# bplaum/gmerlin-avdecoder

Measured on AMD Instinct MI355X. Metric: RTjpeg 1080p decode frames/sec, higher is better.
Workload: dtype i32

## Files before the change

### gmerlin-avdecoder_amd/csrc/mi_rtjpeg.hip

```cpp
#include <hip/hip_runtime.h>
#include <stdarg.h>
#include <stdio.h>
#include <stdlib.h>
#include <string.h>

#include <algorithm>
#include <atomic>
#include <chrono>
#include <condition_variable>
#include <mutex>
#include <string>
#include <thread>
#include <vector>

#include "../../include/mi_rtjpeg.h"
#include "rtj_color_kernels.h"
#include "rtj_common.h"
#include "rtj_decode_chroma.h"
#include "rtj_decode_kernels.h"
#include "rtj_encode_kernels.h"
#include "rtj_format_kernels.h"
#include "rtj_index_kernels.h"
#include "rtj_runs_kernels.h"
#include "rtj_spec_kernels.h"
// ... 63 lines not shown
};

struct SpecIndex {
  bool on = false;
  uint64_t n = 0;
  std::vector<SpecChunkDev> h_chunks;
  std::vector<uint32_t> h_base;
  DevBuf<SpecChunkDev> chunks;
  DevBuf<uint32_t> rec;
  DevBuf<uint32_t> nrec;
  DevBuf<uint32_t> wstart;
  DevBuf<uint2> hand;
  DevBuf<uint2> fix;
  DevBuf<uint8_t> flag;
  DevBuf<uint32_t> nfix;
  DevBuf<uint32_t> base;
  DevBuf<uint32_t> ok;
  DevBuf<uint32_t> todo;
  DevBuf<uint32_t> state;
  uint64_t walkers_cap() const { return flag.cap; }
  uint64_t frames_cap() const { return todo.cap ? todo.cap - 2 : 0; }
};

struct SplitLists {
  DevBuf<uint2> list;
  DevBuf<uint32_t> cnt;
  PinnedBuf<uint32_t> h_mode_seen;
  uint32_t* d_mode_seen = nullptr;
  int flip = 0;
};
// ... 187 lines not shown
  auto spec_chunks_of = [](const FrameDev& f) -> uint32_t { return f.data_len / (uint32_t)kSpecChunk + 1u; };
  for (auto& f : p->h_frames) walkers += spec_chunks_of(f);
  sp.on = !p->sw.serial_index && !p->sw.emit_walk && (p->sw.spec_mode >= 1 || (p->sw.spec_mode != 0 && walkers >= kSpecMinWalkers));
  if (sp.on) {
    sp.h_chunks.clear();
    sp.h_base.assign(1, 0u);
    for (size_t i = 0; i < p->h_frames.size(); i++) {
      const uint32_t nsc = spec_chunks_of(p->h_frames[i]);
      for (uint32_t k = 0; k < nsc; k++) sp.h_chunks.push_back(SpecChunkDev{(uint32_t)i, k});
      sp.h_base.push_back((uint32_t)sp.h_chunks.size());
    }
    sp.n = sp.h_chunks.size();
    if (sp.n >= 0x7FFFFFFFull) sp.on = false;
  }
  if (!sp.on) return MI_RTJ_OK;
  const uint64_t frames = p->h_frames.size();
  if (sp.n > sp.walkers_cap() &&
      ((rc = dev_release(c, s, sp.chunks, sp.rec, sp.nrec, sp.wstart, sp.hand, sp.fix, sp.flag)) || (rc = sp.chunks.grow(c, sp.n, s)) ||
       (rc = sp.rec.grow(c, spec_bits_words(sp.n), s)) || (rc = sp.nrec.grow(c, sp.n, s)) || (rc = sp.wstart.grow(c, sp.n, s)) ||
       (rc = sp.hand.grow(c, sp.n, s)) || (rc = sp.fix.grow(c, sp.n, s)) || (rc = sp.flag.grow(c, sp.n, s, 64, true)) ||
       (rc = sp.nfix.grow(c, 1, s, 0, true))))
    return rc;
  if (frames > sp.frames_cap()) {
    if ((rc = dev_release(c, s, sp.base, sp.ok, sp.todo)) || (rc = sp.base.grow(c, frames + 1, s)) || (rc = sp.ok.grow(c, frames, s, 0, true)) ||
        (rc = sp.todo.grow(c, frames + 2, s)))
      return rc;
    HIPCHK(c, hipMemsetAsync(sp.todo + frames + 1, 0, sizeof(uint32_t), s));
    if ((rc = sp.state.grow(c, kSpecStWords, s, 0, true))) return rc;
  }
  HIPCHK(c, hipMemcpyAsync(sp.chunks, sp.h_chunks.data(), sizeof(SpecChunkDev) * sp.n, hipMemcpyHostToDevice, s));
  HIPCHK(c, hipMemcpyAsync(sp.base, sp.h_base.data(), sizeof(uint32_t) * sp.h_base.size(), hipMemcpyHostToDevice, s));
  HIPCHK(c, hipStreamSynchronize(s));
  return MI_RTJ_OK;
}

int plan_upload(mi_rtj_plan* p) {
  mi_rtj_ctx* c = p->ctx;
  HIPCHK(c, hipSetDevice(c->device));
  const int rc = p->own_frames.grow(c, (uint64_t)p->n, c->stream);
  if (rc != MI_RTJ_OK) return rc;
  p->d_frames = p->own_frames;
  HIPCHK(c, hipMemcpyAsync(p->own_frames, p->h_frames.data(), sizeof(FrameDev) * p->n, hipMemcpyHostToDevice, c->stream));
  return MI_RTJ_OK;
}
// ... 8 lines not shown

int plan_launch(mi_rtj_plan* p, const void* d_stream, void* d_out, int what = kLaunchAll, uint32_t dframe = 0,
                int dcount = -1) {
  mi_rtj_ctx* c = p->ctx;
  Launch L(p, (const uint8_t*)d_stream);
  if (p->fmt != MI_RTJ_FMT_YUV420)
    return launch_fmt(L, dim3(std::min<unsigned>((unsigned)p->n, 16384u)),
                      dim3(kFormats[p->fmt].parts * p->max_groups, (unsigned)p->n), (uint8_t*)d_out);
  int rc;
  if ((rc = launch_open(L, what)) != MI_RTJ_OK) return rc;
  if (what & kLaunchIndex) {
    unsigned rows = (unsigned)p->n;
    const bool spec = p->spec.on && !p->sw.serial_index;
    if (spec) {
      rows = std::min<unsigned>(rows, kSpecFallbackRows);
      const SpecGrids g{dim3((unsigned)((p->spec.n + 63) / 64)), dim3(p->n), dim3(kSpecRepairGrid)};
      if ((rc = stage_spec_index(L, g)) != MI_RTJ_OK) return rc;
    }
    ExactGrids g;
    g.walk = dim3(p->n);
    g.walk_todo = dim3(std::min<unsigned>((unsigned)p->n, 16384u));
    g.summarize = dim3(p->max_chunks, rows);
    g.resolve = dim3(spec ? std::min<unsigned>((unsigned)p->n, 1024u) : rows);
    g.emit = p->sw.emit_walk ? dim3(p->max_chunks, p->n) : dim3(p->max_chunks, rows);
    if ((rc = stage_exact_index(L, g)) != MI_RTJ_OK) return rc;
  }
  if ((rc = launch_hand_over(L, what)) != MI_RTJ_OK) return rc;
  if (!(what & kLaunchDecode)) {
    HIPCHK(c, hipGetLastError());
    return MI_RTJ_OK;
  }
// ... 591 lines not shown
```

### gmerlin-avdecoder_amd/csrc/rtj_host_stages.h

```cpp
#pragma once

namespace {

void drop_events(std::vector<Timed>& v) {
  for (auto& t : v) {
    if (t.a && t.owns_a) (void)hipEventDestroy(t.a);
    if (t.b) (void)hipEventDestroy(t.b);
  }
  v.clear();
}

struct KernelClock {
  mi_rtj_plan* p;
  hipStream_t cur;
  hipEvent_t prev = nullptr;
  Timed t;

  int begin() {
    if (!p->profile) return MI_RTJ_OK;
    t = Timed();
    if (prev) {
      t.a = prev;
      t.owns_a = false;
      return MI_RTJ_OK;
// ... 38 lines not shown
}
void launch_decode_fmt(int fmt, dim3 grid, hipStream_t s, const FrameDev* fr, const uint8_t* st, const QTab* lut, const uint32_t* blk, uint8_t* out) {
  if (fmt == MI_RTJ_FMT_YUV422) hipLaunchKernelGGL(k_decode_fmt<kFmtYUV422>, grid, dim3(kDecThreads), 0, s, fr, st, lut, blk, out);
  else hipLaunchKernelGGL(k_decode_fmt<kFmtGrey>, grid, dim3(kDecThreads), 0, s, fr, st, lut, blk, out);
}

struct WalkArgs {
  const FrameDev* frames;
  const SpecChunkDev* chunks;
  uint32_t total;
  const uint8_t* stream;
  const QTab* lut;
  uint32_t *recbits, *nrec, *wstart;
  uint2* hand;
  SpecReset rs;
};
#define WALK(kernel, ...) \
  hipLaunchKernelGGL(kernel, grid, dim3(64), 0, s, a.frames, a.chunks, a.total, a.stream, a.lut, a.recbits, a.nrec, a.wstart, a.hand, a.rs, ##__VA_ARGS__)
void launch_spec_walk(bool two_types, int spec_mode, uint32_t* state, dim3 grid, hipStream_t s, const WalkArgs& a) {
  if (state) {
    if (!two_types) WALK((k_spec_walk_any<false>), state);
    else WALK((k_spec_walk_any<true>), state);
  } else if (!two_types) {
    if (spec_mode == 1) WALK((k_spec_walk<false, kSpecLead>));
    if (spec_mode == 3) WALK((k_spec_walk<false, kSpecLeadLong>));
    if (spec_mode == 4) WALK((k_spec_walk<false, kSpecLeadVery>));
  } else {
    if (spec_mode == 1) WALK((k_spec_walk<true, kSpecLead>));
    if (spec_mode == 3) WALK((k_spec_walk<true, kSpecLeadLong>));
    if (spec_mode == 4) WALK((k_spec_walk<true, kSpecLeadVery>));
  }
}
#undef WALK

int launch_fmt(Launch& L, dim3 igrid, dim3 dgrid, uint8_t* out) {
  mi_rtj_plan* p = L.p;
  L.c->input_dirty = false;
// ... 33 lines not shown
  return MI_RTJ_OK;
}

struct SpecGrids {
  dim3 walk, verify, repair;
};
int stage_spec_index(Launch& L, const SpecGrids& g) {
  mi_rtj_plan* p = L.p;
  SpecIndex& s = p->spec;
  const QTab* lut = L.c->d_lut;
  const int mode = p->sw.spec_mode;
  const bool no_policy = mode == 1 || mode == 3 || mode == 4;
  L.state = no_policy ? nullptr : s.state.p;
  L.ntodo = s.todo;
  L.todo = s.todo + 1;
  STAGE_CHK(L.clk.begin());
  launch_spec_walk(!p->one_block_type, mode, L.state, g.walk, L.is,
                   WalkArgs{p->d_frames, s.chunks, (uint32_t)s.n, L.st, lut, s.rec, s.nrec, s.wstart, s.hand, SpecReset{s.nfix, s.todo, s.flag}});
  STAGE_CHK(L.clk.end(MI_RTJ_K_SPEC_WALK));
  STAGE_CHK(L.clk.begin());
  for (int pass = 1; pass <= 2; pass++) {
    hipLaunchKernelGGL(k_spec_verify, g.verify, dim3(kSpecVerThreads), 0, L.is, p->d_frames, s.base, lut, s.rec, s.nrec, L.blk,
                       s.ok, s.todo + 1, s.todo, L.state, s.wstart, s.hand, s.fix, s.nfix, s.flag, pass);
    if (pass == 1)
      hipLaunchKernelGGL(k_spec_repair, g.repair, dim3(64), 0, L.is, p->d_frames, s.chunks, L.st, lut, s.rec, s.nrec, s.wstart,
                         s.hand, s.fix, s.nfix, s.flag, (uint32_t)s.n, L.state);
  }
  STAGE_CHK(L.clk.end(MI_RTJ_K_SPEC_VERIFY));
  if (L.state)
    hipLaunchKernelGGL(k_spec_policy, dim3(1), dim3(256), 0, L.is, (uint32_t)p->n, (uint32_t)s.n, s.todo, s.nfix, L.state, p->sw.serial_min);
  return MI_RTJ_OK;
}

struct ExactGrids {
  dim3 walk, walk_todo, summarize, resolve, emit;
};
int stage_exact_index(Launch& L, const ExactGrids& g) {
  mi_rtj_plan* p = L.p;
  const QTab* lut = L.c->d_lut;
  const ChunkIndex& ch = p->chunk;
  if (p->sw.serial_index) {
// ... 151 lines not shown
```

### gmerlin-avdecoder_amd/csrc/rtj_host_switches.h

```cpp
#pragma once
#include <stdint.h>
#include <stdlib.h>
#include <string.h>

namespace mirtj {

static inline const char* exp_env(const char* name) {
#ifdef MIRTJ_EXPERIMENTS
  return getenv(name);
#else
  (void)name;
  return nullptr;
#endif
}

enum PlanKind { kPlanBatch = 0, kPlanOnePacket, kPlanSessionSlot, kPlanSessionGroup };

struct PlanSwitches {
  bool serial_index = false;
  bool emit_walk = false;
  int spec_mode = -1;
  uint32_t dec_slots = 0;
  int rotate = -1;
  uint32_t serial_min = 4096;
  int split = -1;
  bool overlap_set = false;
  int overlap = 0;
};

static inline PlanSwitches plan_switches_from_env(PlanKind kind) {
  PlanSwitches s;
  const char* v = getenv("MI_RTJ_INDEX");
  s.serial_index = v && strcmp(v, "serial") == 0;
  v = getenv("MI_RTJ_EMIT");
  s.emit_walk = v && strcmp(v, "walk") == 0;
  if (kind == kPlanSessionSlot || kind == kPlanSessionGroup) {
    s.spec_mode = 0;
    return s;
  }
  if ((v = getenv("MI_RTJ_SPEC"))) s.spec_mode = atoi(v);
  if (kind != kPlanBatch) return s;
  if ((v = getenv("MI_RTJ_DEC_SLOTS"))) s.dec_slots = (uint32_t)atoi(v);
  if ((v = getenv("MI_RTJ_ROTATE"))) s.rotate = atoi(v) != 0;
  if ((v = getenv("MI_RTJ_SERIAL_MIN"))) s.serial_min = (uint32_t)atoi(v);
  if ((v = getenv("MI_RTJ_SPLIT"))) s.split = atoi(v) != 0;
  if ((v = getenv("MI_RTJ_OVERLAP"))) {
    s.overlap_set = true;
    s.overlap = atoi(v);
  }
  return s;
}

struct LaunchExperiments {
  uint32_t luma_waves = 0, chroma_waves = 0;
  uint32_t xcd_rot = 0;
// ... 50 lines not shown
```

### gmerlin-avdecoder_amd/csrc/rtj_spec_kernels.h

```cpp
#pragma once
#include <hip/hip_runtime.h>

#include "rtj_common.h"
#include "rtj_decode_kernels.h"

#ifndef MIRTJ_SPEC_CHUNK
#define MIRTJ_SPEC_CHUNK 2048
#endif
#ifndef MIRTJ_SPEC_LEAD
#define MIRTJ_SPEC_LEAD 768
#endif

namespace mirtj {

constexpr int kSpecChunk = MIRTJ_SPEC_CHUNK;
constexpr int kSpecLead = MIRTJ_SPEC_LEAD;
#ifndef MIRTJ_SPEC_LEAD_LONG
#define MIRTJ_SPEC_LEAD_LONG 1536
#endif
constexpr int kSpecLeadLong = MIRTJ_SPEC_LEAD_LONG;
#ifndef MIRTJ_SPEC_LEAD_VERY
#define MIRTJ_SPEC_LEAD_VERY 6144
#endif
constexpr int kSpecLeadVery = MIRTJ_SPEC_LEAD_VERY;
constexpr int kSpecSpan = kSpecLeadVery + kSpecChunk;
__host__ __device__ constexpr int spec_lead_of_level(uint32_t level) {
  return level == 0u ? kSpecLead : level == 1u ? kSpecLeadLong : kSpecLeadVery;
}
constexpr int kSpecTile = 128;
constexpr int kSpecTilesMax = kSpecSpan / kSpecTile;
__host__ __device__ constexpr size_t spec_bits_words(uint64_t walkers) {
  return (size_t)((walkers + 1 + 63) / 64) * (size_t)kSpecTilesMax * 64u * 4u;
}
__host__ __device__ constexpr size_t spec_bits_dword(uint32_t walker, uint32_t k) {
  return (((size_t)(walker >> 6) * (size_t)kSpecTilesMax + (k >> 2)) * 64u + (walker & 63u)) * 4u + (k & 3u);
}
constexpr bool spec_bits_layout_ok(uint32_t walkers) {
  const size_t words = spec_bits_words(walkers);
  const uint32_t rows = ((walkers + 1u + 63u) / 64u) * 64u;
  const uint32_t kmax = (uint32_t)kSpecTilesMax * 4u;
  size_t top = 0;
  for (uint32_t w = 0; w < rows; w++) {
    const uint32_t ks[6] = {0u, 3u, 4u, 7u, kmax - 4u, kmax - 1u};
    for (uint32_t k : ks) {
      const size_t d = spec_bits_dword(w, k);
      if (d >= words) return false;
      if (w + 1u < rows && d == spec_bits_dword(w + 1u, k)) return false;
      top = d > top ? d : top;
    }
  }
  const uint32_t ws[3] = {0u, rows > 64u ? 64u : rows - 1u, rows - 1u};
  for (uint32_t w : ws)
    for (uint32_t k = 0; k < kmax; k++) {
      const size_t d = spec_bits_dword(w, k);
      if (d >= words || (k + 1u < kmax && d == spec_bits_dword(w, k + 1u))) return false;
      top = d > top ? d : top;
    }
  return top + 1u == (size_t)rows * kmax && top + 1u <= words;
}
static_assert(spec_bits_layout_ok(1) && spec_bits_layout_ok(63) && spec_bits_layout_ok(64) && spec_bits_layout_ok(65) &&
                  spec_bits_layout_ok(200),
              "a walker's start bits leave the buffer");
constexpr uint64_t kSpecMinWalkers = 40000;
constexpr int kSpecRingRow = 64 + 16;
static_assert(kSpecSpan % kSpecTile == 0 && kSpecSpan < 65536, "walker span: whole tiles, 16-bit positions");
static_assert(kSpecLead >= 6 * 64 + 64 && kSpecLead % kSpecTile == 0 && kSpecChunk % kSpecTile == 0, "the lead: at least one whole macroblock, whole tiles");
static_assert(kSpecLeadLong >= kSpecLead && kSpecLeadLong % kSpecTile == 0 && kSpecLeadVery >= kSpecLeadLong &&
                  kSpecLeadVery % kSpecTile == 0 && kSpecLeadVery % kSpecChunk == 0,
              "leads: whole tiles, growing; the longest a whole number of chunks (a walker that cannot have it starts at byte 0)");

struct SpecChunkDev {
  uint32_t frame;
  uint32_t c;
};
constexpr int kSpecFallbackRows = 64;
constexpr int kSpecRepairGrid = 4096;
constexpr int kSpecPauseLaunches = 64;
enum { kSpecStLost = 0,
       kSpecStPause = 1,
       kSpecStLong = 2,
       kSpecStQuiet = 3,
       kSpecStWords = 4 };
constexpr int kSpecQuietLaunches = 16;
#ifndef MIRTJ_SPEC_VER_THREADS
#define MIRTJ_SPEC_VER_THREADS 512
#endif
#ifndef MIRTJ_SPEC_VER_BATCH
#define MIRTJ_SPEC_VER_BATCH 4
// ... 39 lines not shown
      "v_cmp_lt_i32_e64 %[em], 63, %[u]\n\t"                                                                       \
      "v_max_i32_e32 %[wtn], 1, %[tn]\n\t"                                                                         \
      "s_nop 0\n\t"                                                                                                \
      "v_cndmask_b32_e64 %[u], %[u], 0, %[em]"                                                                     \
      : [u] "+v"(u), [em] "+s"(em), [bits] "+v"(bits_), [tn] "=&v"(tn_), [wtn] "=&v"(wtn_), [wt] "=&v"(wt_),       \
        [wr] "=&v"(wr_), [ma] "=&s"(ma_), [mz] "=&s"(mz_)                                                          \
      : [tm] "v"(tm_), [wtm] "v"(wtm_), [wn] "v"(wn_), [k63] "v"(k63), [kn64] "v"(kn64), [rb] "v"(rb)              \
      : "vcc")

struct SpecReset {
  uint32_t* nfix;
  uint32_t* ntodo;
  uint8_t* fixflag;
};

template <bool PHASE, int LEAD>
__device__ __forceinline__ void spec_walk_body(uint8_t* __restrict__ s_ring, const FrameDev* __restrict__ frames,
                                               const SpecChunkDev* __restrict__ chunks, uint32_t total,
                                               const uint8_t* __restrict__ stream, const QTab* __restrict__ lut,
                                               uint32_t* __restrict__ recbits, uint32_t* __restrict__ nrec,
                                               uint32_t* __restrict__ wstart, uint2* __restrict__ hand,
                                               const SpecReset rs) {
  constexpr int kSpan = LEAD + kSpecChunk;
  static_assert(kSpan % kSpecTile == 0 && kSpan < 65536, "walker span: whole tiles, 16-bit positions");
  const int lane = threadIdx.x;
  const uint32_t g = blockIdx.x * 64u + (uint32_t)lane;
  const bool act = g < total;
  if (act) rs.fixflag[g] = 0;
  if (g == 0u) {
    *rs.nfix = 0u;
    *rs.ntodo = 0u;
  }
  const SpecChunkDev sc = chunks[act ? g : total - 1u];
  const FrameDev f = frames[sc.frame];
  const int lb = lut[f.qidx].lb8 + 1, cb = lut[f.qidx].cb8 + 1;
  const uint32_t cstart = sc.c * (uint32_t)kSpecChunk;
  const uint32_t start = cstart > (uint32_t)LEAD ? cstart - (uint32_t)LEAD : 0u;
  const int take_tile = (int)((cstart - start) / (uint32_t)kSpecTile);
  const int end_tile = take_tile + kSpecChunk / kSpecTile;
  const uint8_t* gp = stream + f.data_off + start;
  const uint32_t sh = (uint32_t)((uintptr_t)gp & 3u);
  const uint32_t* g4 = (const uint32_t*)(gp - sh);
  const int avail = (int)f.data_len - (int)start + (int)sh;

  uint32_t buf[33];
  auto request = [&](int t) {
    const int d0 = t * (kSpecTile / 4);
    if (__all(avail >= 4 * (d0 + 33))) {
#pragma unroll
      for (int k = 0; k < 33; k++) buf[k] = g4[d0 + k];
    } else {
#pragma unroll
      for (int k = 0; k < 33; k++) {
        const int rem = avail - 4 * (d0 + k);
        uint32_t v = 0;
        if (rem > 0) {
          v = g4[d0 + k];
          if (rem < 4) v &= (1u << (8 * rem)) - 1u;
        }
        buf[k] = v;
      }
    }
  };

  int u = 0, rb = lb;
// ... 19 lines not shown
        uint32_t m = dw[j];
        const int c = __builtin_popcount(m);
        if (left >= 0 && left < c) {
          for (int k = 0; k < left; k++) m &= m - 1u;
          const uint32_t pos = (uint32_t)(tile * kSpecTile + 32 * j + 31 - __builtin_ctz(m));
          return ((cnt - 1u - (uint32_t)r) << 16) | pos;
        }
        left -= c;
      }
    }
    return 0u;
  };
  uint32_t take = 0;
  uint32_t tail = 0;
  uint32_t cnt_end = 0;
  uint32_t* const out_bits = recbits + spec_bits_dword(gw, 0);
  uint4 tb = make_uint4(0, 0, 0, 0);

  request(0);
  for (int t = 0; t < kSpan / kSpecTile; t++) {
    if (__any(t == take_tile || t == end_tile)) {
      const uint32_t v = last_aligned_below(t);
      if (t == take_tile) take = sc.c ? v : 0u;
      if (t == end_tile) {
        tail = v;
        cnt_end = cnt;
      }
    }
    uint32_t cur[33];
#pragma unroll
    for (int k = 0; k < 33; k++) cur[k] = buf[k];
    if (t > 0) *(uint4*)(out_bits + (size_t)(t - 1) * 256u) = tb;
    if (t + 1 < kSpan / kSpecTile) request(t + 1);
    int tm_, wtm_;
    {
      const uint32_t w0 = __builtin_amdgcn_alignbyte(cur[1], cur[0], sh);
      tm_ = (int)(int8_t)(w0 & 0xFFu) - 63;
      wtm_ = tm_ > 1 ? tm_ : 1;
    }
    uint32_t bw[4];
#pragma unroll
    for (int i = 0; i < kSpecTile / 16; i++) {
      const uint32_t wd[5] = {__builtin_amdgcn_alignbyte(cur[4 * i + 1], cur[4 * i], sh),
                              __builtin_amdgcn_alignbyte(cur[4 * i + 2], cur[4 * i + 1], sh),
                              __builtin_amdgcn_alignbyte(cur[4 * i + 3], cur[4 * i + 2], sh),
                              __builtin_amdgcn_alignbyte(cur[4 * i + 4], cur[4 * i + 3], sh),
                              i + 1 < kSpecTile / 16 ? __builtin_amdgcn_alignbyte(cur[4 * i + 5], cur[4 * i + 4], sh) : 0u};
      uint32_t bits_ = (i & 1) ? bw[i >> 1] : 0u;
// ... 15 lines not shown
            case 1: MIRTJ_SPEC_STEP1("BYTE_1"); break;
            case 2: MIRTJ_SPEC_STEP1("BYTE_2"); break;
            default: MIRTJ_SPEC_STEP1("BYTE_3"); break;
          }
        }
        tm_ = tn_;
        wtm_ = wtn_;
      }
      bw[i >> 1] = bits_;
    }
    tb = make_uint4(bw[0], bw[1], bw[2], bw[3]);
    ring[t & 3] = tb;
    cnt += (uint32_t)(__builtin_popcount(bw[0]) + __builtin_popcount(bw[1]) + __builtin_popcount(bw[2]) +
                      __builtin_popcount(bw[3]));
  }
  *(uint4*)(out_bits + (size_t)(kSpan / kSpecTile - 1) * 256u) = tb;
  if (end_tile == kSpan / kSpecTile) {
    tail = last_aligned_below(kSpan / kSpecTile);
    cnt_end = cnt;
  }
  if (act) {
    nrec[g] = cnt_end;
    wstart[g] = start;
    hand[g] = make_uint2(take, tail);
  }
}

template <bool PHASE, int LEAD>
__global__ __launch_bounds__(64) void k_spec_walk(const FrameDev* __restrict__ frames,
                                                   const SpecChunkDev* __restrict__ chunks, uint32_t total,
                                                   const uint8_t* __restrict__ stream,
                                                   const QTab* __restrict__ lut, uint32_t* __restrict__ recbits,
                                                   uint32_t* __restrict__ nrec, uint32_t* __restrict__ wstart,
                                                   uint2* __restrict__ hand, const SpecReset rs) {
  __shared__ __attribute__((aligned(16))) uint8_t s_ring[64 * kSpecRingRow];
  spec_walk_body<PHASE, LEAD>(s_ring, frames, chunks, total, stream, lut, recbits, nrec, wstart, hand, rs);
}

template <bool PHASE>
__global__ __launch_bounds__(64) void k_spec_walk_any(const FrameDev* __restrict__ frames,
                                                       const SpecChunkDev* __restrict__ chunks, uint32_t total,
                                                       const uint8_t* __restrict__ stream,
                                                       const QTab* __restrict__ lut, uint32_t* __restrict__ recbits,
                                                       uint32_t* __restrict__ nrec, uint32_t* __restrict__ wstart,
                                                       uint2* __restrict__ hand, const SpecReset rs,
                                                       const uint32_t* __restrict__ state) {
  __shared__ __attribute__((aligned(16))) uint8_t s_ring[64 * kSpecRingRow];
  if (state[kSpecStPause]) return;
  const uint32_t level = state[kSpecStLong];
  if (level == 0u)
    spec_walk_body<PHASE, kSpecLead>(s_ring, frames, chunks, total, stream, lut, recbits, nrec, wstart, hand, rs);
  else if (level == 1u)
    spec_walk_body<PHASE, kSpecLeadLong>(s_ring, frames, chunks, total, stream, lut, recbits, nrec, wstart, hand, rs);
  else
    spec_walk_body<PHASE, kSpecLeadVery>(s_ring, frames, chunks, total, stream, lut, recbits, nrec, wstart, hand, rs);
}

__global__ __launch_bounds__(kSpecVerThreads) void k_spec_verify(const FrameDev* __restrict__ frames,
                                                      const uint32_t* __restrict__ spec_base,
                                                      const QTab* __restrict__ lut,
                                                      const uint32_t* __restrict__ recbits,
                                                      const uint32_t* __restrict__ nrec, uint32_t* __restrict__ blkoff,
                                                      uint32_t* __restrict__ ok, uint32_t* __restrict__ todo,
                                                      uint32_t* __restrict__ ntodo, const uint32_t* __restrict__ state,
                                                      const uint32_t* __restrict__ wstart,
                                                      const uint2* __restrict__ hand, uint2* __restrict__ fix,
                                                      uint32_t* __restrict__ nfix, uint8_t* __restrict__ fixflag, int pass) {
  if (state && state[kSpecStPause]) {
    if (threadIdx.x == 0) ok[blockIdx.x] = 0;
    return;
  }
  if (pass == 2 && ok[blockIdx.x] != 2u) return;
  __shared__ uint32_t s_wave[kSpecVerThreads / 64], s_carry[3];
  __shared__ uint32_t s_i0[kSpecVerThreads], s_base[kSpecVerThreads], s_cnt[kSpecVerThreads];
  __shared__ uint16_t s_pos[kSpecVerThreads / 64][kSpecVerWindow];
  const FrameDev f = frames[blockIdx.x];
  const uint32_t sc0 = spec_base[blockIdx.x], nsc = spec_base[blockIdx.x + 1] - sc0;
  const int tid = threadIdx.x, lane = tid & 63, wv = tid >> 6;
  const uint32_t last = 6u * f.nmb;
  uint32_t* const out = blkoff + f.blk_base;
  if (tid == 0) {
    s_carry[1] = 0;
    s_carry[2] = 0;
  }
  __syncthreads();
  for (uint32_t c0 = 0; c0 < nsc; c0 += kSpecVerThreads) {
    const uint32_t c = c0 + (uint32_t)tid;
    uint32_t cnt = 0, i0 = 0, bad = 0, soft = 0;
    if (c < nsc) {
      const uint32_t n = nrec[sc0 + c];
      const uint2 mine = hand[sc0 + c];
      i0 = c ? mine.x >> 16 : 0u;
      uint32_t i1 = n;
      if (c + 1 < nsc) {
        const uint32_t h = wstart[sc0 + c + 1] + (hand[sc0 + c + 1].x & 0xFFFFu);
        const uint32_t t = wstart[sc0 + c] + (mine.y & 0xFFFFu);
        i1 = mine.y >> 16;
        if (h != t) {
          if (pass == 1 && !bad) {
            soft = 1;
            fix[atomicAdd(nfix, 1u)] = make_uint2(sc0 + c + 1u, t);
            fixflag[sc0 + c + 1u] = 1;
          } else {
            bad = 1;
          }
        }
      }
      if (bad || i1 < i0 || i1 > n) bad = 1;
      else cnt = i1 - i0;
    }
    const uint32_t incl = wave_incl_scan(cnt);
    if (lane == 63) s_wave[wv] = incl;
    const uint32_t anybad = (__any(bad) ? 1u : 0u) | (__any(soft) ? 2u : 0u);
    __syncthreads();
    uint32_t before = s_carry[1] + incl - cnt;
    for (int k = 0; k < wv; k++) before += s_wave[k];
    s_i0[tid] = c < nsc && c ? hand[sc0 + c].x & 0xFFFFu : 0u;
// ... 5 lines not shown
    const uint32_t tile_n = min((uint32_t)kSpecVerThreads, nsc - c0);
    constexpr uint32_t kWaves = kSpecVerThreads / 64;
    static_assert((kSpecChunk + kEntries) / 32 + 2 + 3 <= 128, "two dwords of start bits per lane");
    for (uint32_t j0 = (uint32_t)wv; j0 < tile_n; j0 += kSpecVerBatch * kWaves) {
      uint32_t base[kSpecVerBatch], m[kSpecVerBatch], start[kSpecVerBatch], first[kSpecVerBatch];
      uint32_t w0[kSpecVerBatch], w1[kSpecVerBatch];
#pragma unroll
      for (int u = 0; u < kSpecVerBatch; u++) {
        const uint32_t j = min(j0 + (uint32_t)u * kWaves, tile_n - 1u);
        const bool have = j0 + (uint32_t)u * kWaves < tile_n;
        base[u] = s_base[j];
        m[u] = have && base[u] <= last ? min(s_cnt[j], last + 1u - base[u]) : 0u;
        start[u] = wstart[sc0 + c0 + j];
        first[u] = s_i0[j];
        const uint32_t R = sc0 + c0 + j;
#ifdef MIRTJ_EXP_VER_FROM_ZERO
        w0[u] = m[u] ? recbits[spec_bits_dword(R, (uint32_t)lane)] : 0u;
        w1[u] = m[u] ? recbits[spec_bits_dword(R, (uint32_t)lane + 64u)] : 0u;
        first[u] = c0 + j < nsc && c0 + j ? hand[sc0 + c0 + j].x >> 16 : 0u;
        continue;
#endif
        const uint32_t kt = first[u] >> 5;
        const uint32_t k0 = (kt & ~3u) + (uint32_t)lane, k1 = k0 + 64u;
        w0[u] = m[u] && k0 >= kt && k0 < (uint32_t)(kSpecTilesMax * 4) ? recbits[spec_bits_dword(R, k0)] : 0u;
        w1[u] = m[u] && k1 < (uint32_t)(kSpecTilesMax * 4) ? recbits[spec_bits_dword(R, k1)] : 0u;
        if (k0 == kt) w0[u] &= 0xFFFFFFFFu >> (first[u] & 31u);
      }
#pragma unroll
      for (int u = 0; u < kSpecVerBatch; u++) {
        if (m[u] == 0u) continue;
        const uint32_t c0_ = (uint32_t)__builtin_popcount(w0[u]), c1_ = (uint32_t)__builtin_popcount(w1[u]);
        const uint32_t in0 = wave_incl_scan(c0_);
        const uint32_t tot0 = (uint32_t)__builtin_amdgcn_readlane((int)in0, 63);
        const uint32_t in1 = wave_incl_scan(c1_) + tot0;
        uint32_t* const o = out + base[u];
#ifdef MIRTJ_EXP_VER_FROM_ZERO
        const uint32_t q0 = 32u * (uint32_t)lane, q1 = q0 + 2048u;
#else
        const uint32_t q0 = (first[u] & ~127u) + 32u * (uint32_t)lane, q1 = q0 + 2048u;
#endif
// ... 35 lines not shown
  if (tid == 0) {
    uint32_t v = (s_carry[2] & 1u) ? 0u : (s_carry[2] & 2u) ? 2u : s_carry[1] >= last + 1u ? 1u : 0u;
    ok[blockIdx.x] = v;
    if (!v) todo[atomicAdd(ntodo, 1u)] = blockIdx.x;
  }
}

__global__ __launch_bounds__(64) void k_spec_repair(const FrameDev* __restrict__ frames,
                                                     const SpecChunkDev* __restrict__ chunks,
                                                     const uint8_t* __restrict__ stream,
                                                     const QTab* __restrict__ lut, uint32_t* __restrict__ recbits,
                                                     uint32_t* __restrict__ nrec, uint32_t* __restrict__ wstart,
                                                     uint2* __restrict__ hand, const uint2* __restrict__ fix,
                                                     uint32_t* __restrict__ nfix,
                                                     const uint8_t* __restrict__ fixflag, uint32_t total,
                                                     const uint32_t* __restrict__ state) {
  __shared__ uint32_t s_bits[kSpecTilesMax * 4];
  if (state && state[kSpecStPause]) return;
  const uint32_t n = min(*nfix, total);
  uint32_t extra = 0;
  for (uint32_t i = blockIdx.x; i < n; i += gridDim.x) {
    const uint2 e = fix[i];
    if (fixflag[e.x - 1u]) continue;
    uint32_t w = e.x, from = e.y;
    const uint32_t frame = chunks[w].frame;
    const FrameDev f = frames[frame];
    bool listed = true;
    for (int guard = 0; guard < 4096; guard++) {
      const SpecChunkDev sc = chunks[w];
      const uint32_t limit = (sc.c + 1u) * (uint32_t)kSpecChunk;
      uint32_t take, tail;
      for (int k = threadIdx.x; k < kSpecTilesMax * 4; k += 64) s_bits[k] = 0u;
      __syncthreads();
      const uint32_t cnt = walk_record(f, stream, lut, from, sc.c * (uint32_t)kSpecChunk, limit, s_bits,
                                       (uint32_t)(kSpecTilesMax * 128), take, tail);
      __syncthreads();
      for (int k = threadIdx.x; k < kSpecTilesMax * 4; k += 64) recbits[spec_bits_dword(w, (uint32_t)k)] = s_bits[k];
      __syncthreads();
      if (threadIdx.x == 0) {
        nrec[w] = cnt;
        wstart[w] = from;
        hand[w] = make_uint2(take, tail);
      }
      if (!listed) extra++;
      from += tail & 0xFFFFu;
      if (w + 1u >= total || chunks[w + 1u].frame != frame) break;
      const bool next_listed = fixflag[w + 1u] != 0;
      if (next_listed && !listed) break;
      if (!next_listed && wstart[w + 1u] + (hand[w + 1u].x & 0xFFFFu) == from) break;
      listed = next_listed;
      w++;
    }
  }
  if (threadIdx.x == 0 && extra) atomicAdd(nfix, extra);
}

__global__ __launch_bounds__(256) void k_spec_policy(uint32_t n, uint32_t walkers, uint32_t* __restrict__ todo_cnt,
                                                      const uint32_t* __restrict__ nfix, uint32_t* __restrict__ state,
                                                      const uint32_t serial_min) {
  const uint32_t pause = state[kSpecStPause];
  if (pause) {
    for (uint32_t i = threadIdx.x; i < n; i += 256) todo_cnt[1 + i] = i;
// ... 43 lines not shown
```

Measured before the change: 705,100.

## Walk consecutive speculative chunks as runs to amortize lead-in work

Adds a run mode to the speculative index walk, where one walker covers S consecutive chunks of a frame behind a single lead window instead of one walker per chunk. This is meant to cut the redundant lead-in decoding each chunk walker repeats. Verify and repair are extended to read per-run bit records, map chunks back to their run, and skip re-walking chunks already covered inside a run. The cost is fewer parallel walkers, longer serial work per walker and more bookkeeping (brow, rbase, run bit buffers). Run length is picked automatically from the chunk count, or forced through an environment variable.

```diff
diff --git a/gmerlin-avdecoder_amd/csrc/mi_rtjpeg.hip b/gmerlin-avdecoder_amd/csrc/mi_rtjpeg.hip
--- a/gmerlin-avdecoder_amd/csrc/mi_rtjpeg.hip
+++ b/gmerlin-avdecoder_amd/csrc/mi_rtjpeg.hip
@@ -101,6 +101,14 @@
   DevBuf<uint2> fix;
   DevBuf<uint8_t> flag;
   DevBuf<uint32_t> nfix;
+  uint32_t run_s = 1;
+  uint64_t nruns = 0;
+  std::vector<SpecRunDev> h_runs;
+  std::vector<uint32_t> h_rbase;
+  DevBuf<SpecRunDev> runs;
+  DevBuf<uint32_t> rbase;
+  DevBuf<uint32_t> runrec;
+  DevBuf<uint32_t> brow;
   DevBuf<uint32_t> base;
   DevBuf<uint32_t> ok;
   DevBuf<uint32_t> todo;
@@ -318,6 +326,17 @@
     if (sp.n >= 0x7FFFFFFFull) sp.on = false;
   }
   if (!sp.on) return MI_RTJ_OK;
+  sp.run_s = p->sw.spec_mode == 3 || p->sw.spec_mode == 4 || (p->one_block_type && p->sw.spec_run < 1)
+                 ? 1u
+                 : spec_run_length(sp.n, p->sw.spec_run);
+  sp.h_runs.clear();
+  sp.h_rbase.assign(1, 0u);
+  if (sp.run_s > 1u)
+    for (size_t i = 0; i < p->h_frames.size(); i++) {
+      spec_packet_runs((uint32_t)i, sp.h_base[i], sp.h_base[i + 1] - sp.h_base[i], sp.run_s, sp.h_runs);
+      sp.h_rbase.push_back((uint32_t)sp.h_runs.size());
+    }
+  sp.nruns = sp.h_runs.size();
   const uint64_t frames = p->h_frames.size();
   if (sp.n > sp.walkers_cap() &&
       ((rc = dev_release(c, s, sp.chunks, sp.rec, sp.nrec, sp.wstart, sp.hand, sp.fix, sp.flag)) || (rc = sp.chunks.grow(c, sp.n, s)) ||
@@ -332,6 +351,16 @@
     HIPCHK(c, hipMemsetAsync(sp.todo + frames + 1, 0, sizeof(uint32_t), s));
     if ((rc = sp.state.grow(c, kSpecStWords, s, 0, true))) return rc;
   }
+  if (sp.run_s > 1u) {
+    const uint64_t words = spec_bits_words_t(sp.nruns, spec_run_tiles(sp.run_s));
+    if ((sp.nruns > sp.runs.cap && ((rc = dev_release(c, s, sp.runs)) || (rc = sp.runs.grow(c, sp.nruns, s)))) ||
+        (words > sp.runrec.cap && ((rc = dev_release(c, s, sp.runrec)) || (rc = sp.runrec.grow(c, words, s)))) ||
+        (sp.n > sp.brow.cap && ((rc = dev_release(c, s, sp.brow)) || (rc = sp.brow.grow(c, sp.n, s)))) ||
+        (sp.h_rbase.size() > sp.rbase.cap && ((rc = dev_release(c, s, sp.rbase)) || (rc = sp.rbase.grow(c, sp.h_rbase.size(), s)))))
+      return rc;
+    HIPCHK(c, hipMemcpyAsync(sp.rbase, sp.h_rbase.data(), sizeof(uint32_t) * sp.h_rbase.size(), hipMemcpyHostToDevice, s));
+    HIPCHK(c, hipMemcpyAsync(sp.runs, sp.h_runs.data(), sizeof(SpecRunDev) * sp.nruns, hipMemcpyHostToDevice, s));
+  }
   HIPCHK(c, hipMemcpyAsync(sp.chunks, sp.h_chunks.data(), sizeof(SpecChunkDev) * sp.n, hipMemcpyHostToDevice, s));
   HIPCHK(c, hipMemcpyAsync(sp.base, sp.h_base.data(), sizeof(uint32_t) * sp.h_base.size(), hipMemcpyHostToDevice, s));
   HIPCHK(c, hipStreamSynchronize(s));
@@ -370,7 +399,9 @@
     const bool spec = p->spec.on && !p->sw.serial_index;
     if (spec) {
       rows = std::min<unsigned>(rows, kSpecFallbackRows);
-      const SpecGrids g{dim3((unsigned)((p->spec.n + 63) / 64)), dim3(p->n), dim3(kSpecRepairGrid)};
+      const int sm = p->sw.spec_mode;
+      const uint64_t lanes = p->spec.run_s > 1u && sm == 1 ? p->spec.nruns : p->spec.n;
+      const SpecGrids g{dim3((unsigned)((lanes + 63) / 64)), dim3(p->n), dim3(kSpecRepairGrid)};
       if ((rc = stage_spec_index(L, g)) != MI_RTJ_OK) return rc;
     }
     ExactGrids g;
diff --git a/gmerlin-avdecoder_amd/csrc/rtj_host_stages.h b/gmerlin-avdecoder_amd/csrc/rtj_host_stages.h
--- a/gmerlin-avdecoder_amd/csrc/rtj_host_stages.h
+++ b/gmerlin-avdecoder_amd/csrc/rtj_host_stages.h
@@ -76,13 +76,23 @@
   uint32_t *recbits, *nrec, *wstart;
   uint2* hand;
   SpecReset rs;
+  SpecRunArgs ra;
 };
 #define WALK(kernel, ...) \
-  hipLaunchKernelGGL(kernel, grid, dim3(64), 0, s, a.frames, a.chunks, a.total, a.stream, a.lut, a.recbits, a.nrec, a.wstart, a.hand, a.rs, ##__VA_ARGS__)
+  hipLaunchKernelGGL(kernel, grid, dim3(64), 0, s, a.frames, a.chunks, a.total, a.stream, a.lut, a.recbits, a.nrec, a.wstart, a.hand, a.rs, a.ra, ##__VA_ARGS__)
 void launch_spec_walk(bool two_types, int spec_mode, uint32_t* state, dim3 grid, hipStream_t s, const WalkArgs& a) {
+  const bool runs = a.ra.runs != nullptr;
   if (state) {
-    if (!two_types) WALK((k_spec_walk_any<false>), state);
-    else WALK((k_spec_walk_any<true>), state);
+    if (!two_types) {
+      if (runs) WALK((k_spec_walk_any<false, true>), state);
+      else WALK((k_spec_walk_any<false>), state);
+    } else {
+      if (runs) WALK((k_spec_walk_any<true, true>), state);
+      else WALK((k_spec_walk_any<true>), state);
+    }
+  } else if (runs) {
+    if (!two_types) WALK((k_spec_walk<false, kSpecLead, true>));
+    else WALK((k_spec_walk<true, kSpecLead, true>));
   } else if (!two_types) {
     if (spec_mode == 1) WALK((k_spec_walk<false, kSpecLead>));
     if (spec_mode == 3) WALK((k_spec_walk<false, kSpecLeadLong>));
@@ -146,17 +156,23 @@
   L.state = no_policy ? nullptr : s.state.p;
   L.ntodo = s.todo;
   L.todo = s.todo + 1;
+  const SpecRunArgs ra = s.run_s > 1u ? SpecRunArgs{s.runs.p, (uint32_t)s.nruns, s.run_s, s.runrec.p, s.rbase.p, s.brow.p}
+                                         : SpecRunArgs{nullptr, 0u, 1u, nullptr, nullptr, nullptr};
   STAGE_CHK(L.clk.begin());
   launch_spec_walk(!p->one_block_type, mode, L.state, g.walk, L.is,
-                   WalkArgs{p->d_frames, s.chunks, (uint32_t)s.n, L.st, lut, s.rec, s.nrec, s.wstart, s.hand, SpecReset{s.nfix, s.todo, s.flag}});
+                   WalkArgs{p->d_frames, s.chunks, (uint32_t)s.n, L.st, lut, s.rec, s.nrec, s.wstart, s.hand, SpecReset{s.nfix, s.todo, s.flag}, ra});
   STAGE_CHK(L.clk.end(MI_RTJ_K_SPEC_WALK));
   STAGE_CHK(L.clk.begin());
   for (int pass = 1; pass <= 2; pass++) {
-    hipLaunchKernelGGL(k_spec_verify, g.verify, dim3(kSpecVerThreads), 0, L.is, p->d_frames, s.base, lut, s.rec, s.nrec, L.blk,
-                       s.ok, s.todo + 1, s.todo, L.state, s.wstart, s.hand, s.fix, s.nfix, s.flag, pass);
+    if (ra.runs)
+      hipLaunchKernelGGL(k_spec_verify<true>, g.verify, dim3(kSpecVerThreads), 0, L.is, p->d_frames, s.base, lut, s.rec, s.nrec, L.blk,
+                         s.ok, s.todo + 1, s.todo, L.state, s.wstart, s.hand, s.fix, s.nfix, s.flag, pass, ra);
+    else
+      hipLaunchKernelGGL(k_spec_verify<false>, g.verify, dim3(kSpecVerThreads), 0, L.is, p->d_frames, s.base, lut, s.rec, s.nrec, L.blk,
+                         s.ok, s.todo + 1, s.todo, L.state, s.wstart, s.hand, s.fix, s.nfix, s.flag, pass, ra);
     if (pass == 1)
       hipLaunchKernelGGL(k_spec_repair, g.repair, dim3(64), 0, L.is, p->d_frames, s.chunks, L.st, lut, s.rec, s.nrec, s.wstart,
-                         s.hand, s.fix, s.nfix, s.flag, (uint32_t)s.n, L.state);
+                         s.hand, s.fix, s.nfix, s.flag, (uint32_t)s.n, L.state, ra.brow);
   }
   STAGE_CHK(L.clk.end(MI_RTJ_K_SPEC_VERIFY));
   if (L.state)
diff --git a/gmerlin-avdecoder_amd/csrc/rtj_host_switches.h b/gmerlin-avdecoder_amd/csrc/rtj_host_switches.h
--- a/gmerlin-avdecoder_amd/csrc/rtj_host_switches.h
+++ b/gmerlin-avdecoder_amd/csrc/rtj_host_switches.h
@@ -20,6 +20,7 @@
   bool serial_index = false;
   bool emit_walk = false;
   int spec_mode = -1;
+  int spec_run = 0;
   uint32_t dec_slots = 0;
   int rotate = -1;
   uint32_t serial_min = 4096;
@@ -39,6 +40,7 @@
     return s;
   }
   if ((v = getenv("MI_RTJ_SPEC"))) s.spec_mode = atoi(v);
+  if ((v = getenv("MI_RTJ_SPEC_RUN"))) s.spec_run = atoi(v);
   if (kind != kPlanBatch) return s;
   if ((v = getenv("MI_RTJ_DEC_SLOTS"))) s.dec_slots = (uint32_t)atoi(v);
   if ((v = getenv("MI_RTJ_ROTATE"))) s.rotate = atoi(v) != 0;
diff --git a/gmerlin-avdecoder_amd/csrc/rtj_spec_kernels.h b/gmerlin-avdecoder_amd/csrc/rtj_spec_kernels.h
--- a/gmerlin-avdecoder_amd/csrc/rtj_spec_kernels.h
+++ b/gmerlin-avdecoder_amd/csrc/rtj_spec_kernels.h
@@ -29,31 +29,37 @@
 }
 constexpr int kSpecTile = 128;
 constexpr int kSpecTilesMax = kSpecSpan / kSpecTile;
-__host__ __device__ constexpr size_t spec_bits_words(uint64_t walkers) {
-  return (size_t)((walkers + 1 + 63) / 64) * (size_t)kSpecTilesMax * 64u * 4u;
-}
+__host__ __device__ constexpr size_t spec_bits_words_t(uint64_t walkers, uint32_t tiles) {
+  return (size_t)((walkers + 1 + 63) / 64) * (size_t)tiles * 64u * 4u;
+}
+__host__ __device__ constexpr size_t spec_bits_dword_t(uint32_t walker, uint32_t k, uint32_t tiles) {
+  return (((size_t)(walker >> 6) * (size_t)tiles + (k >> 2)) * 64u + (walker & 63u)) * 4u + (k & 3u);
+}
+__host__ __device__ constexpr size_t spec_bits_words(uint64_t walkers) { return spec_bits_words_t(walkers, (uint32_t)kSpecTilesMax); }
 __host__ __device__ constexpr size_t spec_bits_dword(uint32_t walker, uint32_t k) {
-  return (((size_t)(walker >> 6) * (size_t)kSpecTilesMax + (k >> 2)) * 64u + (walker & 63u)) * 4u + (k & 3u);
-}
-constexpr bool spec_bits_layout_ok(uint32_t walkers) {
-  const size_t words = spec_bits_words(walkers);
+  return spec_bits_dword_t(walker, k, (uint32_t)kSpecTilesMax);
+}
+constexpr int kSpecRunMax = 4;
+__host__ __device__ constexpr uint32_t spec_run_tiles(uint32_t S) { return (uint32_t)(kSpecLead + (int)S * kSpecChunk) / (uint32_t)kSpecTile; }
+constexpr bool spec_bits_layout_ok(uint32_t walkers, uint32_t tiles = (uint32_t)kSpecTilesMax) {
+  const size_t words = spec_bits_words_t(walkers, tiles);
   const uint32_t rows = ((walkers + 1u + 63u) / 64u) * 64u;
-  const uint32_t kmax = (uint32_t)kSpecTilesMax * 4u;
+  const uint32_t kmax = tiles * 4u;
   size_t top = 0;
   for (uint32_t w = 0; w < rows; w++) {
     const uint32_t ks[6] = {0u, 3u, 4u, 7u, kmax - 4u, kmax - 1u};
     for (uint32_t k : ks) {
-      const size_t d = spec_bits_dword(w, k);
+      const size_t d = spec_bits_dword_t(w, k, tiles);
       if (d >= words) return false;
-      if (w + 1u < rows && d == spec_bits_dword(w + 1u, k)) return false;
+      if (w + 1u < rows && d == spec_bits_dword_t(w + 1u, k, tiles)) return false;
       top = d > top ? d : top;
     }
   }
   const uint32_t ws[3] = {0u, rows > 64u ? 64u : rows - 1u, rows - 1u};
   for (uint32_t w : ws)
     for (uint32_t k = 0; k < kmax; k++) {
-      const size_t d = spec_bits_dword(w, k);
-      if (d >= words || (k + 1u < kmax && d == spec_bits_dword(w, k + 1u))) return false;
+      const size_t d = spec_bits_dword_t(w, k, tiles);
+      if (d >= words || (k + 1u < kmax && d == spec_bits_dword_t(w, k + 1u, tiles))) return false;
       top = d > top ? d : top;
     }
   return top + 1u == (size_t)rows * kmax && top + 1u <= words;
@@ -61,6 +67,13 @@
 static_assert(spec_bits_layout_ok(1) && spec_bits_layout_ok(63) && spec_bits_layout_ok(64) && spec_bits_layout_ok(65) &&
                   spec_bits_layout_ok(200),
               "a walker's start bits leave the buffer");
+constexpr bool spec_run_layouts_ok() {
+  for (uint32_t S = 1; S <= (uint32_t)kSpecRunMax; S++)
+    for (uint32_t w : {1u, 63u, 64u, 65u, 200u})
+      if (!spec_bits_layout_ok(w, spec_run_tiles(S))) return false;
+  return true;
+}
+static_assert(spec_run_layouts_ok(), "a run walker's start bits leave the buffer");
 constexpr uint64_t kSpecMinWalkers = 40000;
 constexpr int kSpecRingRow = 64 + 16;
 static_assert(kSpecSpan % kSpecTile == 0 && kSpecSpan < 65536, "walker span: whole tiles, 16-bit positions");
@@ -72,6 +85,33 @@
 struct SpecChunkDev {
   uint32_t frame;
   uint32_t c;
+};
+struct SpecRunDev {
+  uint32_t frame;
+  uint32_t c;
+  uint32_t n;
+  uint32_t chunk;
+};
+template <class Out>
+inline void spec_packet_runs(uint32_t frame, uint32_t chunk0, uint32_t nsc, uint32_t S, Out& out) {
+  for (uint32_t c = 0; c < nsc; c += S) out.push_back(SpecRunDev{frame, c, nsc - c < S ? nsc - c : S, chunk0 + c});
+}
+constexpr uint64_t kSpecGeneration = 256ull * 4ull * 5ull * 64ull;
+constexpr uint64_t kSpecRunMinGens = 4;
+__host__ __device__ constexpr uint32_t spec_run_length(uint64_t chunks, int forced) {
+  if (forced >= 1) return (uint32_t)(forced < kSpecRunMax ? forced : kSpecRunMax);
+  uint32_t S = 1;
+  for (uint32_t k = 2; k <= (uint32_t)kSpecRunMax; k++)
+    if (chunks / k >= kSpecRunMinGens * kSpecGeneration) S = k;
+  return S;
+}
+struct SpecRunArgs {
+  const SpecRunDev* runs;
+  uint32_t nruns;
+  uint32_t S;
+  uint32_t* runbits;
+  const uint32_t* rbase;
+  uint32_t* brow;
 };
 constexpr int kSpecFallbackRows = 64;
 constexpr int kSpecRepairGrid = 4096;
@@ -141,41 +181,72 @@
   uint8_t* fixflag;
 };
 
-template <bool PHASE, int LEAD>
+template <bool PHASE, int LEAD, bool RUNS = false>
 __device__ __forceinline__ void spec_walk_body(uint8_t* __restrict__ s_ring, const FrameDev* __restrict__ frames,
                                                const SpecChunkDev* __restrict__ chunks, uint32_t total,
                                                const uint8_t* __restrict__ stream, const QTab* __restrict__ lut,
                                                uint32_t* __restrict__ recbits, uint32_t* __restrict__ nrec,
                                                uint32_t* __restrict__ wstart, uint2* __restrict__ hand,
-                                               const SpecReset rs) {
+                                               const SpecReset rs, const SpecRunArgs ra) {
   constexpr int kSpan = LEAD + kSpecChunk;
+  constexpr int kChunkTiles = kSpecChunk / kSpecTile;
   static_assert(kSpan % kSpecTile == 0 && kSpan < 65536, "walker span: whole tiles, 16-bit positions");
+  static_assert(!RUNS || LEAD == kSpecLead, "runs are walked behind the short lead only");
+  static_assert(kSpecLead + kSpecRunMax * kSpecChunk < 65536, "a run's span: 16-bit positions and block counts");
   const int lane = threadIdx.x;
   const uint32_t g = blockIdx.x * 64u + (uint32_t)lane;
+  if (RUNS) total = ra.nruns;
+  if (RUNS && blockIdx.x * 64u >= total) return;
   const bool act = g < total;
-  if (act) rs.fixflag[g] = 0;
   if (g == 0u) {
     *rs.nfix = 0u;
     *rs.ntodo = 0u;
   }
-  const SpecChunkDev sc = chunks[act ? g : total - 1u];
+  SpecChunkDev sc;
+  uint32_t nch = 1u, chunk0 = g;
+  if constexpr (RUNS) {
+    const SpecRunDev run = ra.runs[act ? g : total - 1u];
+    sc = SpecChunkDev{run.frame, run.c};
+    nch = act ? run.n : 0u;
+    chunk0 = run.chunk;
+  } else {
+    if (act) rs.fixflag[g] = 0;
+    if (act && ra.brow) ra.brow[g] = 0u;
+    sc = chunks[act ? g : total - 1u];
+  }
   const FrameDev f = frames[sc.frame];
   const int lb = lut[f.qidx].lb8 + 1, cb = lut[f.qidx].cb8 + 1;
   const uint32_t cstart = sc.c * (uint32_t)kSpecChunk;
   const uint32_t start = cstart > (uint32_t)LEAD ? cstart - (uint32_t)LEAD : 0u;
   const int take_tile = (int)((cstart - start) / (uint32_t)kSpecTile);
-  const int end_tile = take_tile + kSpecChunk / kSpecTile;
+  const int end_tile = take_tile + kChunkTiles;
+  const int ntiles = RUNS ? LEAD / kSpecTile + (int)ra.S * kChunkTiles : kSpan / kSpecTile;
+  if constexpr (RUNS) {
+    for (uint32_t j = 0; j < nch; j++) {
+      rs.fixflag[chunk0 + j] = 0;
+      ra.brow[chunk0 + j] = g + 1u;
+      wstart[chunk0 + j] = start;
+    }
+  }
   const uint8_t* gp = stream + f.data_off + start;
   const uint32_t sh = (uint32_t)((uintptr_t)gp & 3u);
   const uint32_t* g4 = (const uint32_t*)(gp - sh);
   const int avail = (int)f.data_len - (int)start + (int)sh;
 
   uint32_t buf[33];
+  bool buf_past = false;
   auto request = [&](int t) {
     const int d0 = t * (kSpecTile / 4);
-    if (__all(avail >= 4 * (d0 + 33))) {
+    buf_past = false;
+    const int left = avail - 4 * d0;
+    if (__all(left >= 4 * 33)) {
 #pragma unroll
       for (int k = 0; k < 33; k++) buf[k] = g4[d0 + k];
+    } else if (__all(left >= 4 * 33 || (left <= 0 && avail >= 4 * 33))) {
+      buf_past = left <= 0;
+      const uint32_t* const src = g4 + (buf_past ? 0 : d0);
+#pragma unroll
+      for (int k = 0; k < 33; k++) buf[k] = src[k];
     } else {
 #pragma unroll
       for (int k = 0; k < 33; k++) {
@@ -225,12 +296,28 @@
   uint32_t take = 0;
   uint32_t tail = 0;
   uint32_t cnt_end = 0;
-  uint32_t* const out_bits = recbits + spec_bits_dword(gw, 0);
+  uint32_t* const out_bits = RUNS ? ra.runbits + spec_bits_dword_t(gw, 0, spec_run_tiles(ra.S)) : recbits + spec_bits_dword(gw, 0);
+  uint32_t* const hand32 = (uint32_t*)hand;
+  auto run_edge = [&](int t) {
+    const int rel = t - take_tile;
+    const bool edge = rel >= 0 && rel % kChunkTiles == 0 && rel / kChunkTiles <= (int)nch;
+    if (!__any(edge)) return;
+    const uint32_t v = last_aligned_below(t);
+    if (!edge) return;
+    const uint32_t j = (uint32_t)(rel / kChunkTiles);
+    if (j > 0u) {
+      hand32[2u * (chunk0 + j - 1u) + 1u] = v;
+      nrec[chunk0 + j - 1u] = cnt;
+    }
+    if (j < nch) hand32[2u * (chunk0 + j)] = sc.c + j ? v : 0u;
+  };
   uint4 tb = make_uint4(0, 0, 0, 0);
 
   request(0);
-  for (int t = 0; t < kSpan / kSpecTile; t++) {
-    if (__any(t == take_tile || t == end_tile)) {
+  for (int t = 0; t < ntiles; t++) {
+    if constexpr (RUNS) {
+      run_edge(t);
+    } else if (__any(t == take_tile || t == end_tile)) {
       const uint32_t v = last_aligned_below(t);
       if (t == take_tile) take = sc.c ? v : 0u;
       if (t == end_tile) {
@@ -239,10 +326,15 @@
       }
     }
     uint32_t cur[33];
-#pragma unroll
-    for (int k = 0; k < 33; k++) cur[k] = buf[k];
+    if (__any(buf_past)) {
+#pragma unroll
+      for (int k = 0; k < 33; k++) cur[k] = buf_past ? 0u : buf[k];
+    } else {
+#pragma unroll
+      for (int k = 0; k < 33; k++) cur[k] = buf[k];
+    }
     if (t > 0) *(uint4*)(out_bits + (size_t)(t - 1) * 256u) = tb;
-    if (t + 1 < kSpan / kSpecTile) request(t + 1);
+    if (t + 1 < ntiles) request(t + 1);
     int tm_, wtm_;
     {
       const uint32_t w0 = __builtin_amdgcn_alignbyte(cur[1], cur[0], sh);
@@ -288,7 +380,11 @@
     cnt += (uint32_t)(__builtin_popcount(bw[0]) + __builtin_popcount(bw[1]) + __builtin_popcount(bw[2]) +
                       __builtin_popcount(bw[3]));
   }
-  *(uint4*)(out_bits + (size_t)(kSpan / kSpecTile - 1) * 256u) = tb;
+  *(uint4*)(out_bits + (size_t)(ntiles - 1) * 256u) = tb;
+  if constexpr (RUNS) {
+    run_edge(ntiles);
+    return;
+  }
   if (end_tile == kSpan / kSpecTile) {
     tail = last_aligned_below(kSpan / kSpecTile);
     cnt_end = cnt;
@@ -300,36 +396,37 @@
   }
 }
 
-template <bool PHASE, int LEAD>
+template <bool PHASE, int LEAD, bool RUNS = false>
 __global__ __launch_bounds__(64) void k_spec_walk(const FrameDev* __restrict__ frames,
                                                    const SpecChunkDev* __restrict__ chunks, uint32_t total,
                                                    const uint8_t* __restrict__ stream,
                                                    const QTab* __restrict__ lut, uint32_t* __restrict__ recbits,
                                                    uint32_t* __restrict__ nrec, uint32_t* __restrict__ wstart,
-                                                   uint2* __restrict__ hand, const SpecReset rs) {
+                                                   uint2* __restrict__ hand, const SpecReset rs, const SpecRunArgs ra) {
   __shared__ __attribute__((aligned(16))) uint8_t s_ring[64 * kSpecRingRow];
-  spec_walk_body<PHASE, LEAD>(s_ring, frames, chunks, total, stream, lut, recbits, nrec, wstart, hand, rs);
-}
-
-template <bool PHASE>
+  spec_walk_body<PHASE, LEAD, RUNS>(s_ring, frames, chunks, total, stream, lut, recbits, nrec, wstart, hand, rs, ra);
+}
+
+template <bool PHASE, bool RUNS = false>
 __global__ __launch_bounds__(64) void k_spec_walk_any(const FrameDev* __restrict__ frames,
                                                        const SpecChunkDev* __restrict__ chunks, uint32_t total,
                                                        const uint8_t* __restrict__ stream,
                                                        const QTab* __restrict__ lut, uint32_t* __restrict__ recbits,
                                                        uint32_t* __restrict__ nrec, uint32_t* __restrict__ wstart,
-                                                       uint2* __restrict__ hand, const SpecReset rs,
+                                                       uint2* __restrict__ hand, const SpecReset rs, const SpecRunArgs ra,
                                                        const uint32_t* __restrict__ state) {
   __shared__ __attribute__((aligned(16))) uint8_t s_ring[64 * kSpecRingRow];
   if (state[kSpecStPause]) return;
   const uint32_t level = state[kSpecStLong];
   if (level == 0u)
-    spec_walk_body<PHASE, kSpecLead>(s_ring, frames, chunks, total, stream, lut, recbits, nrec, wstart, hand, rs);
+    spec_walk_body<PHASE, kSpecLead, RUNS>(s_ring, frames, chunks, total, stream, lut, recbits, nrec, wstart, hand, rs, ra);
   else if (level == 1u)
-    spec_walk_body<PHASE, kSpecLeadLong>(s_ring, frames, chunks, total, stream, lut, recbits, nrec, wstart, hand, rs);
+    spec_walk_body<PHASE, kSpecLeadLong>(s_ring, frames, chunks, total, stream, lut, recbits, nrec, wstart, hand, rs, ra);
   else
-    spec_walk_body<PHASE, kSpecLeadVery>(s_ring, frames, chunks, total, stream, lut, recbits, nrec, wstart, hand, rs);
-}
-
+    spec_walk_body<PHASE, kSpecLeadVery>(s_ring, frames, chunks, total, stream, lut, recbits, nrec, wstart, hand, rs, ra);
+}
+
+template <bool RUNS>
 __global__ __launch_bounds__(kSpecVerThreads) void k_spec_verify(const FrameDev* __restrict__ frames,
                                                       const uint32_t* __restrict__ spec_base,
                                                       const QTab* __restrict__ lut,
@@ -339,7 +436,8 @@
                                                       uint32_t* __restrict__ ntodo, const uint32_t* __restrict__ state,
                                                       const uint32_t* __restrict__ wstart,
                                                       const uint2* __restrict__ hand, uint2* __restrict__ fix,
-                                                      uint32_t* __restrict__ nfix, uint8_t* __restrict__ fixflag, int pass) {
+                                                      uint32_t* __restrict__ nfix, uint8_t* __restrict__ fixflag, int pass,
+                                                      const SpecRunArgs ra) {
   if (state && state[kSpecStPause]) {
     if (threadIdx.x == 0) ok[blockIdx.x] = 0;
     return;
@@ -352,6 +450,7 @@
   const uint32_t sc0 = spec_base[blockIdx.x], nsc = spec_base[blockIdx.x + 1] - sc0;
   const int tid = threadIdx.x, lane = tid & 63, wv = tid >> 6;
   const uint32_t last = 6u * f.nmb;
+  const bool run_walkers = RUNS && (!state || state[kSpecStLong] == 0u);
   uint32_t* const out = blkoff + f.blk_base;
   if (tid == 0) {
     s_carry[1] = 0;
@@ -375,6 +474,10 @@
             soft = 1;
             fix[atomicAdd(nfix, 1u)] = make_uint2(sc0 + c + 1u, t);
             fixflag[sc0 + c + 1u] = 1;
+            if constexpr (RUNS) {
+              if (const uint32_t br = ra.brow[sc0 + c + 1u])
+                for (uint32_t k = 1; k < ra.runs[br - 1u].n; k++) fixflag[sc0 + c + 1u + k] = 2;
+            }
           } else {
             bad = 1;
           }
@@ -410,16 +513,30 @@
         start[u] = wstart[sc0 + c0 + j];
         first[u] = s_i0[j];
         const uint32_t R = sc0 + c0 + j;
+        uint32_t br = 0, first_byte = 0;
+        if constexpr (RUNS) {
+          if (pass == 1 && run_walkers) {
+            const uint32_t r = (c0 + j) / ra.S;
+            br = ra.rbase[blockIdx.x] + r + 1u;
+            first_byte = r ? r * ra.S * (uint32_t)kSpecChunk - (uint32_t)kSpecLead : 0u;
+          } else {
+            br = ra.brow[R];
+            first_byte = start[u];
+          }
+        }
+        const uint32_t* const bits = br ? ra.runbits : recbits;
+        const uint32_t wk = br ? br - 1u : R, tiles = br ? spec_run_tiles(ra.S) : (uint32_t)kSpecTilesMax;
+        const uint32_t kend = br ? min(tiles * 4u, ((c0 + j + 1u) * (uint32_t)kSpecChunk - first_byte + 31u) >> 5) : tiles * 4u;
 #ifdef MIRTJ_EXP_VER_FROM_ZERO
-        w0[u] = m[u] ? recbits[spec_bits_dword(R, (uint32_t)lane)] : 0u;
-        w1[u] = m[u] ? recbits[spec_bits_dword(R, (uint32_t)lane + 64u)] : 0u;
+        w0[u] = m[u] ? bits[spec_bits_dword_t(wk, (uint32_t)lane, tiles)] : 0u;
+        w1[u] = m[u] ? bits[spec_bits_dword_t(wk, (uint32_t)lane + 64u, tiles)] : 0u;
         first[u] = c0 + j < nsc && c0 + j ? hand[sc0 + c0 + j].x >> 16 : 0u;
         continue;
 #endif
         const uint32_t kt = first[u] >> 5;
         const uint32_t k0 = (kt & ~3u) + (uint32_t)lane, k1 = k0 + 64u;
-        w0[u] = m[u] && k0 >= kt && k0 < (uint32_t)(kSpecTilesMax * 4) ? recbits[spec_bits_dword(R, k0)] : 0u;
-        w1[u] = m[u] && k1 < (uint32_t)(kSpecTilesMax * 4) ? recbits[spec_bits_dword(R, k1)] : 0u;
+        w0[u] = m[u] && k0 >= kt && k0 < kend ? bits[spec_bits_dword_t(wk, k0, tiles)] : 0u;
+        w1[u] = m[u] && k1 < kend ? bits[spec_bits_dword_t(wk, k1, tiles)] : 0u;
         if (k0 == kt) w0[u] &= 0xFFFFFFFFu >> (first[u] & 31u);
       }
 #pragma unroll
@@ -485,7 +602,7 @@
                                                      uint2* __restrict__ hand, const uint2* __restrict__ fix,
                                                      uint32_t* __restrict__ nfix,
                                                      const uint8_t* __restrict__ fixflag, uint32_t total,
-                                                     const uint32_t* __restrict__ state) {
+                                                     const uint32_t* __restrict__ state, uint32_t* __restrict__ brow) {
   __shared__ uint32_t s_bits[kSpecTilesMax * 4];
   if (state && state[kSpecStPause]) return;
   const uint32_t n = min(*nfix, total);
@@ -497,7 +614,17 @@
     const uint32_t frame = chunks[w].frame;
     const FrameDev f = frames[frame];
     bool listed = true;
+    uint32_t mark = 1u;
     for (int guard = 0; guard < 4096; guard++) {
+      if (mark == 2u && wstart[w] + (hand[w].x & 0xFFFFu) == from) {
+        from = wstart[w] + (hand[w].y & 0xFFFFu);
+        if (w + 1u >= total || chunks[w + 1u].frame != frame) break;
+        mark = fixflag[w + 1u];
+        if (mark == 0u && wstart[w + 1u] + (hand[w + 1u].x & 0xFFFFu) == from) break;
+        listed = mark != 0u;
+        w++;
+        continue;
+      }
       const SpecChunkDev sc = chunks[w];
       const uint32_t limit = (sc.c + 1u) * (uint32_t)kSpecChunk;
       uint32_t take, tail;
@@ -512,11 +639,13 @@
         nrec[w] = cnt;
         wstart[w] = from;
         hand[w] = make_uint2(take, tail);
-      }
-      if (!listed) extra++;
+        if (brow) brow[w] = 0u;
+      }
+      if (mark != 1u) extra++;
       from += tail & 0xFFFFu;
       if (w + 1u >= total || chunks[w + 1u].frame != frame) break;
-      const bool next_listed = fixflag[w + 1u] != 0;
+      mark = fixflag[w + 1u];
+      const bool next_listed = mark != 0u;
       if (next_listed && !listed) break;
       if (!next_listed && wstart[w + 1u] + (hand[w + 1u].x & 0xFFFFu) == from) break;
       listed = next_listed;
```

Measured after the change: 719,900 (median of 6 runs). 2.1% higher.
